# bcgsc/abyss

Measured on AMD Instinct MI355X. Metric: Mk-mers/s inserted+extended (abyss-bloom-dbg, k=64); unitig bit-exact, higher is better.
Workload: dtype u64

## Files before the change

abyss_amd/csrc/abg_engine.h:

```cpp
#pragma once
#include "abg_walk.h"

#include <algorithm>
#include <chrono>
#include <cstdio>
#include <cstdlib>
#include <cstring>
#include <functional>
#include <future>
#include <string>
#include <type_traits>
#include <vector>

namespace abg {

struct Failure { int code; std::string msg; };
constexpr int FAIL_INVAL = -1, FAIL_NOMEM = -3, FAIL_INTERNAL = -4;
[[noreturn]] inline void fail_now(int code, const std::string& msg) { throw Failure{ code, msg }; }
inline std::string strf(const char* fmt, unsigned long long a = 0, unsigned long long b = 0)
{
	char buf[256];
	snprintf(buf, sizeof buf, fmt, a, b);
	return buf;
}

struct Config {
	uint32_t k = 0, nh = 4, kc = 2, trim = 0;
	uint64_t counters = 0;
	uint32_t cascade_levels = 0;
	std::string spaced_seed;
	uint64_t insert_batch_kmers = 1ull << 24;
	uint32_t claim_log2 = 30;
	uint32_t drain_threshold = 1u << 12;
	uint64_t compact_threshold = 1u << 20;
	bool async_load = true;
	bool tiled_insert = true;
	bool benign_sharers = true;
	uint32_t cls_debug_skip = 0;
	bool cls_archive = true;
	uint32_t cls_archive_max_mb = 16384;
	bool sorted_overflow = true;
	bool cosettle = true;
	uint32_t cosettle_passes = 6;
	uint32_t cosettle_log2 = 24;
	uint32_t walk_slots = 4096;
	uint32_t tb_cap = 512;
	uint32_t buf_cap = 1u << 16;
	uint64_t pool_cap = 1ull << 28;
	uint32_t rec_cap = 1u << 22;
	uint32_t wtab_log2 = 26;
	uint32_t wtab_log2_max = 31;
	uint32_t cend_log2 = 20;
	uint64_t p2_first_batch = 65536;
	uint64_t p2_max_batch = 1ull << 22;
	uint32_t p2_growth = 2;
	uint32_t p2_crowded = 1u << 18;
	uint32_t p2_starved_growth = 2;
	uint32_t p2_starved = 6144;
	uint32_t slice_filter = 0;
	bool solid_plane = true;
	uint32_t classify_slots = 0;
	uint32_t cls_both_max_mb = 1024;
	bool cls_both = true;
	bool prefetch_classify = true;
	uint32_t memo_log2 = 0;
	bool memo = true;
	uint32_t p2_max_candidates = 1u << 18;
	uint32_t t_tags = 1024;
	uint32_t commit_incremental = 1;
	uint32_t commit_dirty_max = 4096;
	uint32_t commit_dirty_log2 = 26;
	uint32_t guide_stride = 4;
	uint32_t guide_log2_max = 31;
	bool guide_seen = true;
	bool link_duplicates = true;
	bool par_commit = true;
	bool overlap_bins = true;
	bool overlap_purity = true;
	bool apply_mask = true;
	bool lead_implicit = true;
	uint32_t dist_hash_all_ranks = 2;
	uint32_t dist_route_min_ranks = 4;
	uint64_t keep_insert_scratch_bytes = 16ull << 30;
	uint64_t par_commit_max_bytes = 16ull << 30;
	int verbose = 0;
};

struct Counters {
	uint64_t solid_reads = 0, visited_reads = 0, reads_processed = 0, bases_assembled = 0,
	         contig_id = 0;
};

struct BaseCodes {
	uint8_t t[256];
	BaseCodes()
	{
		for (int i = 0; i < 256; i++) t[i] = 0xFF;
		t['A'] = t['a'] = 0; t['C'] = t['c'] = 1; t['G'] = t['g'] = 2; t['T'] = t['t'] = 3;
	}
};
template <class T>
struct NoInitAlloc : std::allocator<T> {
	template <class U> struct rebind { using other = NoInitAlloc<U>; };
	template <class U, class... A> void construct(U* p, A&&... a)
	{
		if constexpr (sizeof...(A) == 0) ::new ((void*)p) U; else ::new ((void*)p) U(std::forward<A>(a)...);
	}
};
struct HostBatch {
	std::vector<uint32_t, NoInitAlloc<uint32_t>> words;
	std::vector<uint64_t> woff{ 0 };
	std::vector<uint32_t> len;
	std::vector<uint64_t> koff{ 0 };
	void clear() { words.clear(); woff.assign(1, 0); len.clear(); koff.assign(1, 0); }
	uint64_t n() const { return len.size(); }
	void add_ascii(const char* s, uint32_t L, uint32_t k)
	{
		static const BaseCodes codes;
		uint64_t w0 = words.size();
		words.resize(w0 + (L + 15) / 16);
		uint32_t* out = words.data() + w0;
		uint32_t i = 0;
		for (; i + 16 <= L; i += 16) {
			uint32_t w = 0;
			for (uint32_t j = 0; j < 16; j++) w |= (uint32_t)(codes.t[(unsigned char)s[i + j]] & 3u) << (2 * j);
			*out++ = w;
		}
		if (i < L) {
// ... 2604 lines not shown
						both_set(e.both32, pos);
						if (e.cnt8) { const unsigned c = e.cnt8[pos]; mn = c < mn ? c : mn; }
					}
					if (e.cnt8) cov += mn;
				}
				if (cov) atomic_add_u32(&rec.coverage, cov);
			}
		}
		if (lane == 0) { e.cnt[i] = nrec; e.cnt2[i] = nins; e.cnt3[i] = bases; }
	}
};
struct FPcCover {
	ParCommit e; uint8_t* kmin; uint32_t sum;
	ABG_HDN void operator()(uint64_t i, uint32_t lane, uint32_t nlanes) const
	{
		const uint32_t c = e.c_begin + (uint32_t)i;
		if (c >= e.brk || !e.active[i]) return;
		for (uint32_t ri = e.first_rec[c]; ri != REC_END; ri = e.recs[ri].next) {
			ContigRec& rec = e.recs[ri];
			if (!rec.ins) continue;
			const uint64_t* ch = e.kh + rec.seq_off;
			const uint32_t cnk = rec.len - e.p.k + 1;
			uint32_t cov = 0;
			for (uint32_t j = lane; j < cnk; j += nlanes) {
				if (sum) { cov += kmin[rec.seq_off + j]; continue; }
				const uint64_t h = ch[j];
				unsigned mn = 255;
				for (unsigned q = 0; q < e.p.nh; q++) {
					const uint64_t pos = pos_i(e.p, h, q);
					if (pos - e.own_lo < e.own_span) { const unsigned v = e.cnt8[pos]; mn = v < mn ? v : mn; }
				}
				kmin[rec.seq_off + j] = (uint8_t)mn;
			}
			if (sum && cov) atomic_add_u32(&rec.coverage, cov);
		}
	}
};
struct FPcWrite {
	ParCommit e; uint32_t* order; uint32_t order_base; uint64_t id_base;
	ABG_HD void operator()(uint64_t i, uint32_t) const
	{
		const uint32_t c = e.c_begin + (uint32_t)i;
		if (c >= e.brk || !e.active[i]) return;
		uint32_t o = order_base + e.cnt[i];
		uint64_t id = id_base + e.cnt2[i];
		for (uint32_t ri = e.first_rec[c]; ri != REC_END; ri = e.recs[ri].next) {
			ContigRec& rec = e.recs[ri];
			order[o++] = ri;
			if (rec.ins) rec.contig_id = id++;
		}
	}
};

constexpr uint32_t CLS_SLOTS_SMALL = 65536;
template <class BE> auto classify_lanes(BE& be, int) -> decltype(be.classify_lanes()) { return be.classify_lanes(); }
template <class BE> uint32_t classify_lanes(BE&, long) { return CLS_SLOTS_SMALL; }
template <class BE> auto device_mem_free(BE& be, int) -> decltype(be.device_mem_free()) { return be.device_mem_free(); }
template <class BE> uint64_t device_mem_free(BE&, long) { return 0; }
template <class BE>
class Engine {
  public:
	Engine(BE& be, const Config& cfg) : be_(be), cfg_(cfg)
	{
		uint64_t rem = cfg_.counters % 8;
		m_ = rem ? cfg_.counters + 8 - rem : cfg_.counters;
		p_ = make_params(cfg_.k, cfg_.nh, cfg_.kc, cfg_.trim, m_);
		if (!cfg_.spaced_seed.empty()) {
			MaskTab* mt = new MaskTab;
			make_mask(cfg_.spaced_seed.c_str(), cfg_.k, *mt, p_);
			mask_d_ = (MaskTab*)be_.alloc(sizeof(MaskTab));
			be_.h2d(mask_d_, mt, sizeof(MaskTab));
			delete mt;
			p_.mask = mask_d_;
		}
		if (cfg_.cascade_levels) {
			casc_.levels = cfg_.cascade_levels;
			casc_.level_words = (m_ + 31) / 32;
			casc_.bits = (uint32_t*)be_.alloc(casc_.levels * casc_.level_words * 4);
			be_.memset(casc_.bits, 0, casc_.levels * casc_.level_words * 4);
			cnt_ = (uint8_t*)be_.alloc(8);
			vis_bytes_ = 8;
		} else {
			const uint64_t dev = be_.device_mem_bytes();
			cnt_deferred_ = cfg_.slice_filter == 1 || (cfg_.slice_filter == 0 && dev && (double)m_ * 1.3 > (double)dev * 0.9);
			if (!cnt_deferred_) {
				cnt_ = (uint8_t*)be_.alloc(m_ + 64 * (MAX_RANKS + 1));
				be_.memset(cnt_, 0, m_);
			}
			vis_bytes_ = (m_ / 8 + 4 + 3) & ~3ull;
		}
		vis_ = (uint8_t*)be_.alloc(vis_bytes_);
		be_.memset(vis_, 0, vis_bytes_);
		cstate_ = (CommitState*)be_.alloc(sizeof(CommitState));
		be_.memset(cstate_, 0, sizeof(CommitState));
		scal_ = (uint64_t*)be_.alloc(64);
	}
	~Engine()
	{
		if (BE::ITEM_GROUP_LOG2 == 0 && getenv("ABG_LEAD_COUNT"))
			fprintf(stderr, "lead_stores made=%llu skipped=%llu\n", (unsigned long long)stats_.lead_stores[0], (unsigned long long)stats_.lead_stores[1]);
		free_counters(); be_.free(vis_); if (both_) be_.free(both_); be_.free(cstate_); be_.free(scal_);
		free_archive();
		if (casc_.bits) be_.free(casc_.bits);
		if (mask_d_) be_.free(mask_d_);
		if (T_) be_.free(T_);
		if (Tk_) { be_.free(Tk_); be_.free(Tv_); }
// ... 379 lines not shown
		mark("batches");
		deliveries_wait();
		be_.sync_side();
		mark("last delivery");
		pre_n_ = 0; prefetch_ = nullptr;
		guide_.tab = nullptr;
		be_.free(result_d);
	}
	void ensure_memo()
	{
		if (!cfg_.memo) { memo_.k0 = nullptr; return; }
		if (!memo_tab_.hmin) {
			uint32_t log2 = cfg_.memo_log2;
			if (!log2) { log2 = 16; while (log2 < 26 && (1ull << log2) < m_ / 128) log2++; }
			alloc_tab(memo_tab_, log2);
			memo_valid_ = false; plane_valid_ = false;
		}
		if (!memo_valid_) {
			be_.memset(memo_tab_.hmin, 0xFF, (memo_tab_.mask + 1) * 8);
			be_.memset(memo_tab_.hmax, 0xFF, (memo_tab_.mask + 1) * 8);
			be_.memset(memo_tab_.meta, 0, (memo_tab_.mask + 1) * 8);
			memo_valid_ = true;
			memo_gen_++;
		}
		memo_ = SuccMemo{ memo_tab_.hmin, memo_tab_.hmax, memo_tab_.meta, memo_tab_.mask };
	}
	void ensure_plane()
	{
		p2_ = p_; cnt2_ = cnt_;
		if (!cfg_.solid_plane || casc_.bits || (m_ & 63)) return;
		if (!plane_) plane_ = (uint8_t*)be_.alloc((sliced_ ? (uint64_t)comm_.world * own_chunk_ : m_) / 8 + 64);
		if (!plane_valid_ && sliced_) {
			FSolidPlane f{ (const uint64_t*)(cnt_ + own_lo_), p_.kc, (uint64_t*)(plane_ + own_lo_ / 8) };
			be_.launch(own_span_ / 64, f, "solid_plane");
			std::vector<uint64_t> c(comm_.world), d(comm_.world);
			for (int q = 0; q < comm_.world; q++) { d[q] = (uint64_t)q * (own_chunk_ / 8); c[q] = own_chunk_ / 8; }
			c_all_gather_v(plane_, c.data(), d.data());
			plane_valid_ = true; cnt_partial_ = false;
		} else if (!plane_valid_) {
			FSolidPlane f{ (const uint64_t*)cnt_, p_.kc, (uint64_t*)plane_ };
			be_.launch(m_ / 64, f, "solid_plane");
			plane_valid_ = true;
		}
		p2_.solid_bits = 1; cnt2_ = plane_;
	}
	void ensure_both()
	{
		const bool want = cfg_.cls_both && p2_.solid_bits && !dist() && !sliced_ && !(m_ & 63) && m_ / 4 <= ((uint64_t)cfg_.cls_both_max_mb << 20);
		if (!want) { if (both_) { be_.free(both_); both_ = nullptr; } return; }
		if (!both_) both_ = (uint8_t*)be_.try_alloc(m_ / 4 + 64);
		if (!both_) return;
		FBothBuild f{ (const uint32_t*)plane_, (const uint32_t*)vis_, (uint64_t*)both_ };
		be_.launch(m_ / 32, f, "both_build");
	}
	uint8_t* both_ = nullptr;
	void free_archive()
	{
		if (arc_.seq) { be_.free(arc_.seq); be_.free(arc_.used); be_.free(arc_.tab); }
		arc_ = ContigArchive(); arc_valid_ = false;
	}
	void ensure_archive(const Batch& b)
	{
		const bool want = cfg_.cls_archive && !dist() && !sliced_ && !casc_.bits && b.n && use_par_commit();
		if (!want) { free_archive(); return; }
		const uint64_t nk = loaded_ops_ ? loaded_ops_ : m_ / 4;
		uint64_t cap = std::max<uint64_t>(nk / 4, 1ull << 16) + ARC_HEAD, slots = 1ull << 12;
		while (slots < cap / 2) slots <<= 1;
		const uint64_t budget = (uint64_t)cfg_.cls_archive_max_mb << 20;
		while (slots > (1ull << 12) && slots * 8 + cap > budget) { slots >>= 1; cap = std::min(cap, slots * 2); }
		if (cap >= (1ULL << ARC_POS_BITS)) cap = (1ULL << ARC_POS_BITS) - 1;
		if (arc_.seq && (arc_.cap < cap || arc_.mask + 1 < slots)) free_archive();
		if (!arc_.seq) {
			arc_.seq = (uint8_t*)be_.try_alloc(cap + ARC_PAD);
			arc_.tab = (uint64_t*)be_.try_alloc(slots * 8);
			arc_.used = (uint64_t*)be_.try_alloc(8);
			if (!arc_.seq || !arc_.tab || !arc_.used) {
				if (arc_.seq) be_.free(arc_.seq); if (arc_.tab) be_.free(arc_.tab); if (arc_.used) be_.free(arc_.used);
				arc_ = ContigArchive();
				return;
			}
			arc_.cap = cap; arc_.mask = slots - 1;
			arc_valid_ = false;
		}
		arc_.nreads = wstats_ ? wstats_ + WSTAT_CLS_COVERED : nullptr;
		if (!arc_valid_) {
			be_.memset(arc_.seq, ARC_SEP, arc_.cap + ARC_PAD);
			be_.memset(arc_.tab, 0, (arc_.mask + 1) * 8);
			const uint64_t head = ARC_HEAD;
			be_.h2d(arc_.used, &head, 8);
			arc_valid_ = true;
		}
	}
	ContigArchive arc_{}; bool arc_valid_ = false;
	uint64_t loaded_ops_ = 0;
	uint64_t ovf_seen_[2] = { 0, 0 };
	uint8_t* plane_ = nullptr; bool plane_valid_ = false;
	Params p2_; const uint8_t* cnt2_ = nullptr;

	void build_guide(const Batch& b)
	{
		guide_.tab = nullptr; guide_.seen = nullptr; guide_slots_ = 0;
		if (!cfg_.guide_stride || p_.nh > 8 || !b.n) return;
		const uint64_t sampled = (b.n + cfg_.guide_stride - 1) / cfg_.guide_stride;
		uint64_t nwords = 0;
		be_.d2h(&nwords, b.woff + b.n, 8);
		const uint64_t bases = nwords * 16, minus = b.n * (uint64_t)(p_.k - 1);
		const uint64_t kmers = (bases > minus ? bases - minus : b.n) / std::min<uint32_t>(cfg_.guide_stride, 4u);
		uint32_t log2 = 16;
// ... 851 lines not shown
		free_tab(wtab_);
		wtab_log2_++;
		alloc_tab(wtab_, wtab_log2_);
		be_.free(pool_); be_.free(kh_);
		pool_cap_ *= 2;
		pool_ = (uint8_t*)be_.alloc(pool_cap_);
		kh_ = (uint64_t*)be_.alloc(pool_cap_ * 8);
		if (cfg_.verbose)
			fprintf(stderr, "abyss_amd: walker resources grown: %u frames, %u bases, 2^%u table, %llu pool\n",
			    walk_tb_cap_, walk_buf_cap_, wtab_log2_, (unsigned long long)pool_cap_);
	}

	template <int NW>
	WalkEnv<NW> make_env(const Batch& b, uint32_t* cand_d, uint32_t* status_d, uint32_t* first_d)
	{
		WalkEnv<NW> e;
		e.p = p2_; e.cnt = cnt2_; e.batch = b; e.cand_read = cand_d; e.status = status_d; e.first_rec = first_d;
		e.tab = wtab_; e.owner_base = 0;
		e.tb_pool = (TBFrame<NW>*)tb_pool_;
		e.tbk_pool = tbk_pool_;
		e.tb_cap = walk_tb_cap_;
		e.fast = nullptr; e.fast_bytes = 0; e.dbg = dbg_; e.coop = false;
		e.la_pool = la_pool_;
		e.guide = guide_; e.bulk_pool = bulk_pool_; e.wstats = wstats_; e.memo = memo_; e.mcache = nullptr;
		e.lbuf_pool = lbuf_; e.rbuf_pool = rbuf_; e.buf_cap = walk_buf_cap_;
		e.pool = pool_; e.pool_cap = pool_cap_; e.pool_used = pool_used_;
		e.recs = recs_; e.rec_cap = rec_cap_; e.rec_used = rec_used_;
		return e;
	}

	template <int NW>
	uint32_t commit(const Batch& b, uint32_t* cand_d, uint32_t* status_d, uint32_t* first_d,
	    uint8_t* result_d, const uint64_t* rkoff_d, uint32_t c_begin, uint32_t c_end)
	{
		{
			uint32_t nrec = 0, nord = 0;
			be_.d2h(&nrec, rec_used_, 4);
			be_.d2h(&nord, order_n_, 4);
			uint64_t need = cend_count_ + 2ull * (std::min(nrec, rec_cap_) - std::min(nord, rec_cap_));
			while (need * 2 > cend_.mask + 1) grow_cend();
		}
		CommitState cs;
		cs.counters = counters_;
		cs.break_at = c_begin; cs.pad_ = 0; cs.cend_count = cend_count_;
		be_.h2d(cstate_, &cs, sizeof cs);
		{
			FPreCommit<NW> f{ p_, b, cand_d, status_d, first_d, recs_, vis_, kh_, rkh_, rkoff_d, read_flag_, c_begin, 0, ~0ULL, nullptr, nullptr, nullptr };
			be_.launch_wave(c_end - c_begin, f, "precommit");
			FPreCommitCopies fc{ status_d, first_d, recs_, read_flag_, c_begin, p_.k };
			be_.launch(c_end - c_begin, fc, "precommit");
		}
		CommitEnv<NW> e;
		e.read_flag = read_flag_;
		e.p = p_; e.b = b; e.vis32 = (uint32_t*)vis_; e.both32 = (uint32_t*)both_;
		e.cand_read = cand_d; e.status = status_d; e.first_rec = first_d;
		e.recs = recs_; e.pool = pool_; e.result = result_d;
		e.kh = kh_; e.rkh = rkh_; e.rkoff = rkoff_d;
		e.cend = cend_; e.st = cstate_;
		e.order = order_; e.order_n = order_n_;
		be_.template launch_commit<NW>(e, c_begin, c_end);
		be_.d2h(&cs, cstate_, sizeof cs);
		counters_ = cs.counters;
		cend_count_ = cs.cend_count;
		if (cs.pad_) fail_now(FAIL_INTERNAL, "contigEndKmers table overflowed");
		return cs.break_at;
	}

	template <int NW>
	uint32_t commit_par(const Batch& b, uint32_t* cand_d, uint32_t* status_d, uint32_t* first_d,
	    uint8_t* result_d, uint64_t* rkoff_d, uint32_t c_begin, uint32_t c_end)
	{
		uint32_t n = c_end - c_begin;
		const uint32_t n0 = n;
		uint32_t nrec = 0, nord = 0;
		be_.d2h(&nrec, rec_used_, 4);
		be_.d2h(&nord, order_n_, 4);
		nrec = std::min(nrec, rec_cap_);
		{
			uint64_t need = cend_count_ + 2ull * (nrec - std::min(nord, rec_cap_));
			while (need * 2 > cend_.mask + 1) grow_cend();
		}
		const bool part = dist();
		uint8_t* part_buf = part ? (uint8_t*)be_.alloc((uint64_t)n + nrec + 64) : nullptr;
		uint8_t* part_c = part_buf; uint8_t* part_r = part ? part_buf + n : nullptr;
		uint32_t* nfirst = part ? nullptr : (uint32_t*)be_.alloc(n * 4ull + 4);
		if (nfirst) be_.memset(nfirst, 0, n * 4ull);
		{
			if (part) be_.memset(part_buf, 1, (uint64_t)n + nrec);
			FPreCommit<NW> f{ p_, b, cand_d, status_d, first_d, recs_, vis_, kh_, rkh_, rkoff_d, read_flag_, c_begin,
				part ? own_lo_ : 0, part ? own_span_ : ~0ULL, part_c, part_r, nfirst };
			be_.launch_wave(n, f, "precommit");
			if (!part) { FPreCommitCopies fc{ status_d, first_d, recs_, read_flag_, c_begin, p_.k }; be_.launch(n, fc, "precommit"); }
			if (part) {
				c_all_reduce(part_buf, (uint64_t)n + nrec, DT_U8, OP_MIN);
				FPreCommitFin ff{ status_d, first_d, recs_, read_flag_, c_begin, p_.k, part_c, part_r };
				be_.launch(n, ff, "precommit");
			}
		}
		ParCommit e;
		e.own_lo = part ? own_lo_ : 0; e.own_span = part ? own_span_ : ~0ULL; e.part_c = part_c; e.part_r = part_r;
		e.p = p_; e.b = b; e.cand_read = cand_d; e.status = status_d; e.first_rec = first_d;
		e.recs = recs_; e.pool = pool_; e.result = result_d; e.kh = kh_; e.rkh = rkh_; e.rkoff = rkoff_d;
		e.read_flag = read_flag_; e.vis32 = (uint32_t*)vis_; e.both32 = (uint32_t*)both_; e.T = T_; e.cend = cend_; e.cnt8 = cnt_;
		if (!part) e.arc = arc_;
		e.Tk = nullptr; e.Tv = nullptr; e.Tmask = 0;
		if (t_hashed()) {
			uint64_t bases = 0;
			be_.d2h(&bases, pool_used_, 8);
			const uint64_t need = std::min<uint64_t>(bases, pool_cap_) * p_.nh + 16;
			if (!Tk_ || (T_entries_ + need) * 2 > (1ull << Tlog2_)) {
				uint32_t log2 = 20;
				while ((1ull << log2) < 2 * need) log2++;
				if (!Tk_ || log2 > Tlog2_) {
					if (Tk_) { be_.free(Tk_); be_.free(Tv_); }
					Tlog2_ = log2;
					Tk_ = (uint64_t*)be_.alloc(8ull << Tlog2_);
					Tv_ = (uint32_t*)be_.alloc(4ull << Tlog2_);
				}
				be_.memset(Tk_, 0xFF, 8ull << Tlog2_);
				be_.memset(Tv_, 0xFF, 4ull << Tlog2_);
				T_entries_ = 0;
				t_tag_ = std::min<uint32_t>(cfg_.t_tags, T_TAGS) - 1;
			}
			T_entries_ += need;
			e.T = nullptr; e.Tk = Tk_; e.Tv = Tv_; e.Tmask = (1ull << Tlog2_) - 1;
		}
		e.c_begin = c_begin; e.c_end = c_end; e.brk = c_end;
		e.off = (uint32_t*)be_.alloc((n + 1ull) * 4); e.cnt = (uint32_t*)be_.alloc(n * 4ull + 4);
		e.cnt2 = (uint32_t*)be_.alloc(n * 4ull + 4); e.cnt3 = (uint64_t*)be_.alloc(n * 8ull + 8);
		e.active = (uint8_t*)be_.alloc(n + 8ull); e.short_list = (uint32_t*)be_.alloc(nrec * 4ull + 4);
		e.scal = (uint32_t*)be_.alloc(64);
		uint32_t scal_h[8] = { 0, 0xFFFFFFFFu, 0, 0, 0, 0, 0, 0 };
		be_.h2d(e.scal, scal_h, sizeof scal_h);
		e.nfirst = nfirst;
		const bool incremental = cfg_.commit_incremental && (cfg_.commit_incremental > 1 || !t_hashed()) && !part && cfg_.commit_dirty_max > 0 && nrec > 0;
		uint32_t* dirty_buf = nullptr;
		e.dirty = nullptr; e.dirty_cap = 0; e.A = nullptr; e.A_shift = 0;
		if (incremental) {
			e.dirty_cap = (uint32_t)std::min<uint64_t>(std::min(cfg_.commit_dirty_max, 8192u), std::max(nrec, 1u));
			dirty_buf = (uint32_t*)be_.alloc(2ull * e.dirty_cap * 4 + 8);
			e.dirty = dirty_buf;
			if (!pcA_) {
				const uint32_t log2 = std::min(34u, std::max(10u, cfg_.commit_dirty_log2));
				pcA_bits_ = std::min<uint64_t>(m_, 1ull << log2);
				pcA_shift_ = pcA_bits_ < m_ ? 64 - log2 : 0;
				pcA_ = (uint32_t*)be_.alloc((pcA_bits_ + 31) / 32 * 4 + 4);
				be_.memset(pcA_, 0, (pcA_bits_ + 31) / 32 * 4 + 4);
			}
			e.A = pcA_; e.A_shift = pcA_shift_;
		}
		e.tcend = WalkTab{ nullptr, nullptr, nullptr, 0 };
		std::vector<uint32_t> c1(n), c2(n), off(n + 1ull);
		{ FPcCount f{ e }; be_.launch(n, f, "pc_count"); }
		be_.d2h(c1.data(), e.cnt, n * 4ull);
		off[0] = 0;
		for (uint32_t i = 0; i < n; i++) off[i + 1] = off[i] + c1[i];
// ... 241 lines not shown
		if (log2 == wtab_log2_) return;
		free_tab(wtab_);
		wtab_log2_ = log2;
		alloc_tab(wtab_, wtab_log2_);
		if (cfg_.verbose) fprintf(stderr, "abyss_amd: walker vertex table grown to 2^%u entries\n", wtab_log2_);
	}
	uint32_t wtab_log2_cap()
	{
		uint32_t cap = cfg_.wtab_log2_max;
		const uint64_t mem = be_.device_mem_bytes();
		while (mem && cap > cfg_.wtab_log2 && (24ull << cap) > mem / 8) cap--;
		return cap;
	}
	void clear_wtab()
	{
		be_.memset(wtab_.hmin, 0xFF, (wtab_.mask + 1) * 8);
		be_.memset(wtab_.meta, 0xFF, (wtab_.mask + 1) * 8);
	}

	struct BatchRun {
		Batch v{};
		uint64_t first = 0, n = 0;
		uint8_t* res_d = nullptr;
		std::vector<uint32_t> cand_h;
		uint32_t nc = 0;
		uint32_t* cand_d = nullptr; uint32_t* status_d = nullptr; uint32_t* first_d = nullptr;
		uint32_t* need_d = nullptr; uint32_t* need_n = nullptr; uint64_t* rkoff_d = nullptr;
		uint32_t base = 0;
		uint32_t prepped = 0, owner_next = 0, committed = 0, force = 0xFFFFFFFFu, nneed = 0, nneed_all = 0;
		bool round_started = false;
		bool predicted = false;
		bool pending = false;
		bool overflow = false, debug = false;
	};
	template <int NW>
	void assemble_nw(const Batch& b, uint8_t* result_d, uint8_t* results_host,
	    const std::function<void(const ContigOut&)>& sink)
	{
		uint64_t next = 0;
		while (next < b.n) {
			ensure_walk();
			BatchRun r;
			classify_batch<NW>(b, next, std::min<uint64_t>(p2_batch_, b.n - next), result_d, r);
			next += r.n;
			counters_.reads_processed += r.n;
			p2_batch_ = next_batch_size();
			prefetch_ = nullptr;
			if (next < b.n && !dist() && cfg_.prefetch_classify) {
				const uint64_t nf = next, nn = std::min<uint64_t>(p2_batch_, b.n - next);
				prefetch_ = [this, &b, result_d, nf, nn]() {
					if (!la_pool_c2_) la_pool_c2_ = (VKey*)be_.alloc((uint64_t)cslots_ * LA_MAX_VISITED * sizeof(VKey));
					Batch vn = b;
					vn.woff = b.woff + nf; vn.len = b.len + nf; vn.koff = b.koff + nf; vn.n = nn;
					FClassify<NW> f{ p2_, vn, 0, cnt2_, vis_, result_d + nf, la_pool_c2_, both_, arc_, cfg_.cls_debug_skip };
					be_.launch_slots_side(nn, f, cslots_, "classify");
					pre_first_ = nf; pre_n_ = nn;
				};
			}
			if (r.nc) {
				setup_batch<NW>(r);
				finish_batch<NW>(r, sink);
			}
			if (results_host) {
				be_.d2h(results_host + r.first, r.res_d, r.n);
				if (const void* left = memchr(results_host + r.first, RES_CANDIDATE, r.n)) {
					fail_now(FAIL_INTERNAL, strf("read %llu left unprocessed", (unsigned long long)((const uint8_t*)left - results_host)));
				}
			}
		}
	}

	template <int NW>
	void classify_batch(const Batch& b, uint64_t first, uint64_t n, uint8_t* result_d, BatchRun& r)
	{
		Batch v = b;
		v.woff = b.woff + first; v.len = b.len + first; v.koff = b.koff + first; v.n = n;
		uint8_t* res_d = result_d + first;
		if (!la_pool_c_) la_pool_c_ = (VKey*)be_.alloc((uint64_t)cslots_ * LA_MAX_VISITED * sizeof(VKey));
		if (pre_n_ == n && pre_first_ == first) {
			const auto t_wait = std::chrono::steady_clock::now();
			be_.sync_side();
			stats_.cls_wait_ms += std::chrono::duration<double, std::milli>(std::chrono::steady_clock::now() - t_wait).count();
			FRefilter<NW> f{ p_, v, vis_, res_d };
			be_.launch(n, f, "reclassify");
		} else if (dist()) {
			const uint64_t R = (uint64_t)comm_.world;
			std::vector<uint64_t> c(R), d(R);
			for (uint64_t q = 0; q < R; q++) { d[q] = n * q / R; c[q] = n * (q + 1) / R - d[q]; }
			FClassify<NW> f{ p2_, v, d[comm_.rank], cnt2_, vis_, res_d, la_pool_c_ };
			be_.launch_slots(c[comm_.rank], f, cslots_, "classify");
			c_all_gather_v(res_d, c.data(), d.data());
		} else {
			be_.sync_side();
			FClassify<NW> f{ p2_, v, 0, cnt2_, vis_, res_d, la_pool_c_, both_, arc_, cfg_.cls_debug_skip };
			be_.launch_slots(n, f, cslots_, "classify");
		}
		pre_n_ = 0;
		std::vector<uint8_t> res(n);
		be_.d2h(res.data(), res_d, n);
		r = BatchRun();
		uint64_t used = n;
		const uint64_t max_cand = std::min<uint64_t>(cfg_.p2_max_candidates,
		    std::max<uint64_t>(1024, (1ull << wtab_log2_cap()) / (2 * wtab_per_walker_)));
		for (const uint8_t* q = res.data(), *end = q + n; (q = (const uint8_t*)memchr(q, RES_CANDIDATE, (size_t)(end - q))) != nullptr; q++) {
			if (r.cand_h.size() >= max_cand) { used = (uint64_t)(q - res.data()); break; }
			r.cand_h.push_back((uint32_t)(q - res.data()));
		}
		uint64_t n_visited = 0;
		for (uint64_t i = 0; i < used; i++) n_visited += res[i] == RR_ALL_KMERS_VISITED;
		counters_.solid_reads += n_visited + r.cand_h.size();
		counters_.visited_reads += n_visited;
		v.n = used;
		r.v = v; r.first = first; r.n = used; r.res_d = res_d;
		r.nc = (uint32_t)r.cand_h.size();
		if (used < n) stats_.batch_cuts++;
		stats_.candidates += r.nc;
		last_candidates_ = r.nc;
	}

	template <int NW>
	void setup_batch(BatchRun& r)
	{
		const uint32_t nc = r.nc;
		const Batch& b = r.v;
		r.cand_d = (uint32_t*)be_.alloc(nc * 4ull);
		r.status_d = (uint32_t*)be_.alloc(nc * 4ull);
		r.first_d = (uint32_t*)be_.alloc(nc * 4ull);
		r.need_d = (uint32_t*)be_.alloc(nc * 4ull);
		r.need_n = (uint32_t*)be_.alloc(8);
		be_.h2d(r.cand_d, r.cand_h.data(), nc * 4ull);
		std::vector<uint32_t> len_h(nc);
		{
			uint32_t* cl = (uint32_t*)be_.alloc(nc * 4ull + 4);
			FGatherU32 f{ b.len, r.cand_d, cl };
			be_.launch(nc, f, "gather_len");
			be_.d2h(len_h.data(), cl, nc * 4ull);
			be_.free(cl);
		}
		std::vector<uint64_t> rkoff(nc + 1, 0);
		for (uint32_t i = 0; i < nc; i++) rkoff[i + 1] = rkoff[i] + (len_h[i] - p_.k + 1);
		r.rkoff_d = (uint64_t*)be_.alloc((nc + 1) * 8ull);
		be_.h2d(r.rkoff_d, rkoff.data(), (nc + 1) * 8ull);
		rkh_ = (uint64_t*)be_.alloc(std::max<uint64_t>(rkoff[nc], 1) * 8);
		read_flag_ = (uint8_t*)be_.alloc(nc);
		{
			FReadPrep<NW> f{ p_, b, r.cand_d, r.rkoff_d, rkh_, 0 };
// ... 210 lines not shown
```

abyss_amd/csrc/abg_host.h:

```cpp
#pragma once
#include "abg_engine.h"
#include "../../include/abyss_amd.h"

#include <cctype>
#include <cmath>
#include <map>
#include <string>
#include <atomic>
#include <chrono>
#include <future>
#include <memory>
#include <thread>

namespace abg {
static_assert(FAIL_NOMEM == ABG_ENOMEM && FAIL_INTERNAL == ABG_EINTERNAL, "Failure codes are the C ABI's");


struct FContainsSolid {
	Params p; const uint64_t* h0; const uint8_t* cnt; uint8_t* out;
	ABG_HD void operator()(uint64_t t, uint32_t) const { out[t] = solid_contains(p, cnt, h0[t]) ? 1 : 0; }
};
struct FExpand {
	Params p; const uint64_t* h0; uint64_t* out;
	ABG_HD void operator()(uint64_t t, uint32_t) const
// ... 23 lines not shown
	explicit Session(A&&... a) : be(std::forward<A>(a)...) {}
	~Session() { try { drain(); } catch (...) {} keep_drop(false); delete eng; }

	int create(const abg_params& p)
	{
		if (p.k < 2 || p.k > ABG_MAX_KMER) return fail(ABG_EINVAL, "k must be in 2.." + std::to_string(ABG_MAX_KMER));
		if (p.num_hashes < 1 || p.num_hashes > ABG_MAX_HASHES) return fail(ABG_EINVAL, "num_hashes must be in 1..32");
		if (p.spaced_seed && p.spaced_seed[0]) {
			std::string m(p.spaced_seed);
			if (m.size() != p.k) return fail(ABG_EINVAL, "spaced seed must be exactly k bits long");
			if (m.find_first_not_of("01") != std::string::npos) return fail(ABG_EINVAL, "spaced seed must contain only '0's or '1's");
			if (m.front() != '1' || m.back() != '1') return fail(ABG_EINVAL, "spaced seed must begin and end with '1's");
			if (!std::equal(m.begin(), m.end(), m.rbegin())) return fail(ABG_EINVAL, "spaced seed must be symmetric");
			if (m.find('0') != std::string::npos) cfg.spaced_seed = m;
		}
		cfg.k = p.k; cfg.nh = p.num_hashes; cfg.kc = p.min_cov;
		cfg.trim = (p.trim == 0xFFFFFFFFu) ? p.k : p.trim;
		cfg.counters = p.counters ? p.counters : counters_for_budget(p.bloom_bytes);
		cfg.cascade_levels = p.cascade_levels;
		cfg.slice_filter = p.slice_filter;
		if (const char* e = getenv("ABG_SLICE_FILTER")) cfg.slice_filter = (uint32_t)atoi(e);
		if (p.cascade_levels && (!p.counters || p.counters % 64)) return fail(ABG_EINVAL, "cascade mode needs `counters` = bits per level, a multiple of 64");
		if (!cfg.counters) return fail(ABG_EINVAL, "bloom_bytes / counters must be > 0");
		cfg.verbose = p.verbose;
		if (p.insert_batch_kmers) cfg.insert_batch_kmers = p.insert_batch_kmers;
		if (p.claim_log2) cfg.claim_log2 = p.claim_log2;
		if (p.walk_slots) cfg.walk_slots = p.walk_slots;
		if (p.wtab_log2) cfg.wtab_log2 = p.wtab_log2;
		if (const char* e = getenv("ABG_CLAIM_LOG2")) cfg.claim_log2 = (uint32_t)atoi(e);
		if (const char* e = getenv("ABG_INSERT_BATCH")) cfg.insert_batch_kmers = strtoull(e, 0, 10);
		if (const char* e = getenv("ABG_WALK_SLOTS")) cfg.walk_slots = (uint32_t)atoi(e);
		if (const char* e = getenv("ABG_WTAB_LOG2")) cfg.wtab_log2 = (uint32_t)atoi(e);
		if (const char* e = getenv("ABG_WTAB_LOG2_MAX")) cfg.wtab_log2_max = (uint32_t)std::max<int>(atoi(e), (int)cfg.wtab_log2);
		if (const char* e = getenv("ABG_POOL_CAP")) cfg.pool_cap = std::max<uint64_t>(1024, strtoull(e, 0, 10));
		if (const char* e = getenv("ABG_REC_CAP")) cfg.rec_cap = (uint32_t)std::max(16, atoi(e));
		if (const char* e = getenv("ABG_P2_FIRST_BATCH")) cfg.p2_first_batch = strtoull(e, 0, 10);
		if (const char* e = getenv("ABG_P2_MAX_BATCH")) cfg.p2_max_batch = strtoull(e, 0, 10);
		if (const char* e = getenv("ABG_PAR_COMMIT")) cfg.par_commit = atoi(e) != 0;
		if (const char* e = getenv("ABG_T_TAGS")) cfg.t_tags = (uint32_t)std::max(2, atoi(e));
		if (const char* e = getenv("ABG_COMMIT_INCREMENTAL")) cfg.commit_incremental = (uint32_t)std::min(2, std::max(0, atoi(e)));
		if (const char* e = getenv("ABG_COMMIT_DIRTY_MAX")) cfg.commit_dirty_max = (uint32_t)std::max(0, atoi(e));
		if (const char* e = getenv("ABG_COMMIT_DIRTY_LOG2")) cfg.commit_dirty_log2 = (uint32_t)std::min(34, std::max(10, atoi(e)));
		if (const char* e = getenv("ABG_PAR_COMMIT_MAX_GB")) cfg.par_commit_max_bytes = strtoull(e, 0, 10) << 30;
		if (const char* e = getenv("ABG_COMPACT_THRESHOLD")) cfg.compact_threshold = strtoull(e, 0, 10);
		if (const char* e = getenv("ABG_TILED")) cfg.tiled_insert = atoi(e) != 0;
		if (const char* e = getenv("ABG_DIST_ROUTE_MIN")) cfg.dist_route_min_ranks = (uint32_t)atoi(e);
		if (const char* e = getenv("ABG_BENIGN")) cfg.benign_sharers = atoi(e) != 0;
		if (const char* e = getenv("ABG_CLS_ARCHIVE")) cfg.cls_archive = atoi(e) != 0;
		if (const char* e = getenv("ABG_CLS_DEBUG_SKIP")) cfg.cls_debug_skip = (uint32_t)atoi(e);
		if (const char* e = getenv("ABG_CLS_ARCHIVE_MAX_MB")) cfg.cls_archive_max_mb = (uint32_t)std::max(0, atoi(e));
		if (const char* e = getenv("ABG_SORTED_OVERFLOW")) cfg.sorted_overflow = atoi(e) != 0;
		if (const char* e = getenv("ABG_COSETTLE")) cfg.cosettle = atoi(e) != 0;
		if (const char* e = getenv("ABG_CLS_BOTH")) cfg.cls_both = atoi(e) != 0;
		if (const char* e = getenv("ABG_CLS_BOTH_MAX_MB")) cfg.cls_both_max_mb = (uint32_t)std::max(0, atoi(e));
		if (const char* e = getenv("ABG_COSETTLE_PASSES")) cfg.cosettle_passes = (uint32_t)std::max(1, atoi(e));
		if (const char* e = getenv("ABG_COSETTLE_LOG2")) cfg.cosettle_log2 = (uint32_t)std::min(25, std::max(5, atoi(e)));
		if (const char* e = getenv("ABG_LINK_DUPS")) cfg.link_duplicates = atoi(e) != 0;
		if (const char* e = getenv("ABG_OVERLAP_PURITY")) cfg.overlap_purity = atoi(e) != 0;
		if (const char* e = getenv("ABG_LEAD_IMPLICIT")) cfg.lead_implicit = atoi(e) != 0;
		if (const char* e = getenv("ABG_APPLY_MASK")) cfg.apply_mask = atoi(e) != 0;
		if (const char* e = getenv("ABG_OVERLAP_BINS")) cfg.overlap_bins = atoi(e) != 0;
		if (const char* e = getenv("ABG_PREFETCH")) cfg.prefetch_classify = atoi(e) != 0;
		if (const char* e = getenv("ABG_ASYNC_LOAD")) cfg.async_load = atoi(e) != 0;
		if (const char* e = getenv("ABG_CLS_SLOTS")) cfg.classify_slots = (uint32_t)std::max(64, atoi(e));
		if (const char* e = getenv("ABG_SOLID_PLANE")) cfg.solid_plane = atoi(e) != 0;
		if (const char* e = getenv("ABG_MEMO")) cfg.memo = atoi(e) != 0;
		if (const char* e = getenv("ABG_P2_MAX_CANDIDATES")) cfg.p2_max_candidates = (uint32_t)std::max(1, atoi(e));
		if (const char* e = getenv("ABG_P2_STARVED_GROWTH")) cfg.p2_starved_growth = (uint32_t)std::max(2, atoi(e));
		if (const char* e = getenv("ABG_P2_STARVED")) cfg.p2_starved = (uint32_t)atoi(e);
		if (const char* e = getenv("ABG_P2_GROWTH")) cfg.p2_growth = (uint32_t)std::max(2, atoi(e));
		if (const char* e = getenv("ABG_DRAIN_THRESHOLD")) cfg.drain_threshold = (uint32_t)strtoul(e, 0, 10);
		if (const char* e = getenv("ABG_GUIDE_STRIDE")) cfg.guide_stride = (uint32_t)strtoul(e, 0, 10);
		if (const char* e = getenv("ABG_GUIDE_SEEN")) cfg.guide_seen = atoi(e) != 0;
		if (const char* e = getenv("ABG_GUIDE_LOG2_MAX")) cfg.guide_log2_max = (uint32_t)std::min(36, std::max(10, atoi(e)));
		if (!be.ok()) return fail(ABG_ENODEV, be.why());
		eng = new Engine<BE>(be, cfg);
		return ABG_OK;
	}

	int load_seqs(const char* seqs, const uint64_t* off, uint64_t n) { return load_seqs_v(1, &seqs, &off, &n); }
	int load_seqs_v(uint32_t nchunks, const char* const* seqs_v, const uint64_t* const* off_v, const uint64_t* n_v)
	{
		const uint32_t k = cfg.k;
		const double t_call = std::chrono::duration<double>(std::chrono::steady_clock::now().time_since_epoch()).count();
		const uint32_t max_piece = (uint32_t)std::min<uint64_t>(1u << 20, cfg.insert_batch_kmers + k - 1);
		struct Part { uint32_t c; uint64_t a, b; };
		std::vector<Part> plan;
		std::vector<uint64_t> base(nchunks + 1, 0);
		for (uint32_t c = 0; c < nchunks; c++) {
			base[c + 1] = base[c] + n_v[c];
			if (!n_v[c]) continue;
			const std::vector<uint64_t> cut = split_reads(off_v[c], n_v[c]);
			for (size_t t = 0; t + 1 < cut.size(); t++) plan.push_back(Part{ c, cut[t], cut[t + 1] });
		}
		const bool keeping = keep_on_ && !keep_failed_;
		std::vector<KeptPart> kparts(keeping ? plan.size() : 0);
		std::vector<uint8_t> verdict(keeping ? base[nchunks] : 0, (uint8_t)RR_UNINITIALIZED);
		std::vector<HostBatch> parts(plan.size());
		const bool timing = getenv("ABG_HOST_TIMING") != nullptr;
		const auto tnow = []() { return std::chrono::duration<double>(std::chrono::steady_clock::now().time_since_epoch()).count(); };
		const double t0 = tnow();
		run_parts(parts.size(), [&](size_t t) {
			HostBatch& hb = parts[t];
			const Part& pt = plan[t];
			const char* seqs = seqs_v[pt.c];
			const uint64_t* off = off_v[pt.c];
// ... 721 lines not shown
```

abyss_amd/csrc/abg_kernels.hip:

```cpp
#include <hip/hip_runtime.h>
#include <hip/hip_ext.h>
#include <hipcub/hipcub.hpp>
#include <rccl/rccl.h>
#include <dlfcn.h>
#include <unistd.h>

#include "abg_host.h"
#include "abg_overlap.h"

#include <chrono>
#include <map>
#include <mutex>

namespace {

template <class F>
__global__ void __launch_bounds__(256) k_foreach(F f, uint64_t n)
{
	uint64_t i = (uint64_t)blockIdx.x * blockDim.x + threadIdx.x;
	const uint64_t stride = (uint64_t)gridDim.x * blockDim.x;
	const uint32_t slot = (uint32_t)i;
	for (; i < n; i += stride) f(i, slot);
}
#ifndef ABG_CLS_WAVES
// ... 137 lines not shown
struct ProfEntry { double ms = 0; uint64_t launches = 0; };

struct HipBackend {
	static constexpr uint32_t ITEM_GROUP_LOG2 = 6;
	int device = 0;
	bool good = false;
	std::string reason;
	hipStream_t stream = nullptr;
	hipStream_t stream2 = nullptr;
	hipEvent_t ev2a = nullptr, ev2b = nullptr;
	std::string side_name;
	bool side_pending = false;
	bool profiling = false;
	std::map<std::string, ProfEntry> prof;
	uint32_t cus = 256;
	unsigned long long* ticket = nullptr;

	explicit HipBackend(int dev = 0) : device(dev)
	{
		int n = 0;
		hipError_t e = hipGetDeviceCount(&n);
		if (e != hipSuccess || n <= 0) { reason = "no HIP device available (abyss_amd has no CPU fallback)"; return; }
		if (dev < 0 || dev >= n) { reason = "HIP device ordinal out of range"; return; }
		if (hipSetDevice(dev) != hipSuccess) { reason = "hipSetDevice failed"; return; }
		hipDeviceProp_t prop;
		if (hipGetDeviceProperties(&prop, dev) == hipSuccess) cus = (uint32_t)prop.multiProcessorCount;
		if (hipStreamCreate(&stream) != hipSuccess) { reason = "hipStreamCreate failed"; return; }
		if (const char* e = getenv("ABG_MEM_LIMIT_MB")) mem_limit = (size_t)strtoull(e, 0, 10) << 20;
		if (const char* e = getenv("ABG_CLS_TICKETS")) cls_tickets = atoi(e) != 0;
		{
			int lo = 0, hi = 0;
			hipDeviceGetStreamPriorityRange(&lo, &hi);
			const char* e = getenv("ABG_SIDE_PRIORITY");
			const bool low = !e || atoi(e) != 0;
			if (hipStreamCreateWithPriority(&stream2, hipStreamNonBlocking, low ? lo : hi) != hipSuccess) { reason = "hipStreamCreate failed"; return; }
		}
		hipEventCreate(&ev2a);
		hipEventCreate(&ev2b);
		good = true;
	}
	~HipBackend()
	{
		if (ticket) free(ticket);
		if (cls_ticket_) free(cls_ticket_);
		if (pin) hipHostFree(pin);
		for (int i = 0; i < 2; i++) { if (big_pin[i]) hipHostFree(big_pin[i]); if (big_ev[i]) hipEventDestroy(big_ev[i]); }
		for (int i = 0; i < 2; i++) { if (ahead_pin[i]) hipHostFree(ahead_pin[i]); if (ahead_ev[i]) hipEventDestroy(ahead_ev[i]); if (ahead[i].dev) hipFree(ahead[i].dev); }
		for (void* q : ahead_old) hipFree(q);
		if (ahead_stream) hipStreamDestroy(ahead_stream);
		if (cub_tmp) hipFree(cub_tmp);
		drop_cache();
		prof_drain(true);
		for (auto& q : prof_free) { hipEventDestroy(q.first); hipEventDestroy(q.second); }
		if (ev2a) hipEventDestroy(ev2a);
		if (ev2b) hipEventDestroy(ev2b);
		if (stream2) hipStreamDestroy(stream2);
		if (stream) hipStreamDestroy(stream);
	}
	bool ok() const { return good; }
	std::string why() const { return reason; }
	void bind_thread() { (void)hipSetDevice(device); }
	static void check(hipError_t e, const char* what)
	{
		if (e != hipSuccess) {
			(void)hipGetLastError();
			abg::fail_now(e == hipErrorOutOfMemory ? abg::FAIL_NOMEM : abg::FAIL_INTERNAL, std::string(what) + " failed: " + hipGetErrorString(e));
		}
	}
	static constexpr size_t CACHE_MAX_BLOCK = 256ull << 20, CACHE_MAX_TOTAL = 8ull << 30;
	std::map<size_t, std::vector<void*>> cache_free;
	std::map<void*, size_t> cache_size;
	size_t cache_held = 0;
	size_t mem_limit = 0, mem_used = 0;
	std::map<void*, size_t> mem_size;
	hipError_t dev_malloc(void** p, size_t n)
	{
		if (mem_limit && mem_used + n > mem_limit) return hipErrorOutOfMemory;
		const hipError_t e = hipMalloc(p, n);
		if (e == hipSuccess && mem_limit) { mem_used += n; mem_size[*p] = n; }
		return e;
	}
	void dev_free(void* p)
	{
		if (mem_limit) { auto it = mem_size.find(p); if (it != mem_size.end()) { mem_used -= it->second; mem_size.erase(it); } }
		hipFree(p);
	}
	void* try_alloc(size_t n)
	{
		void* p = nullptr;
		hipSetDevice(device);
		if (dev_malloc(&p, n ? n : 1) != hipSuccess) { (void)hipGetLastError(); return nullptr; }
		if (getenv("ABG_MEM_DEBUG")) fprintf(stderr, "[mem] +%.2f GB (optional)\n", n / 1e9);
		return p;
	}
	void* alloc(size_t n)
	{
		void* p = nullptr;
		hipSetDevice(device);
		if (n > CACHE_MAX_BLOCK) {
			hipError_t e = dev_malloc(&p, n);
			if (e != hipSuccess) {
				(void)hipGetLastError();
				drop_cache();
				e = dev_malloc(&p, n);
			}
			if (e != hipSuccess) out_of_memory(n);
// ... 273 lines not shown
	{
		if (!n) return;
		uint64_t blocks = (n + 255) / 256;
		uint64_t cap = (uint64_t)cus * 8;
		if (blocks > cap) blocks = cap;
		launch_kernel(name, k_foreach<F>, dim3((uint32_t)blocks), dim3(256), f, n);
	}
	template <class F>
	void launch_slots(uint64_t n, F f, uint32_t slots, const char* name)
	{
		if (!n) return;
		uint64_t blocks = (n + 63) / 64;
		uint64_t cap = slots / 64 ? slots / 64 : 1;
		if (blocks > cap) blocks = cap;
		if (!cls_tickets) { launch_kernel(name, k_foreach_w<F>, dim3((uint32_t)blocks), dim3(64), f, n); return; }
		unsigned long long* t = cls_ticket(0);
		check(hipMemsetAsync(t, 0, 8, stream), "hipMemsetAsync");
		launch_kernel(name, k_foreach_wt<F>, dim3((uint32_t)blocks), dim3(64), f, n, t);
	}
	bool cls_tickets = true;
	unsigned long long* cls_ticket_ = nullptr;
	unsigned long long* cls_ticket(int side)
	{
		if (!cls_ticket_) cls_ticket_ = (unsigned long long*)alloc(256);
		return cls_ticket_ + (side ? 16 : 0);
	}
	uint32_t classify_lanes() const { return cus * 4 * ABG_CLS_WAVES * 64; }
	uint64_t device_mem_free() const
	{
		size_t fr = 0, tot = 0;
		if (hipMemGetInfo(&fr, &tot) != hipSuccess) { (void)hipGetLastError(); return 0; }
		if (mem_limit) fr = std::min(fr, mem_limit > mem_used ? mem_limit - mem_used : (size_t)0);
		return fr;
	}
	template <class F>
	void launch_slots_side(uint64_t n, F f, uint32_t slots, const char* name)
	{
		if (!n) return;
		uint64_t blocks = (n + 63) / 64;
		uint64_t cap = slots / 64 ? slots / 64 : 1;
		if (blocks > cap) blocks = cap;
		hipEventRecord(ev2a, stream);
		hipStreamWaitEvent(stream2, ev2a, 0);
		unsigned long long* t = cls_tickets ? cls_ticket(1) : nullptr;
		if (t) check(hipMemsetAsync(t, 0, 8, stream2), "hipMemsetAsync");
		hipEventRecord(ev2a, stream2);
		if (t) hipLaunchKernelGGL(k_foreach_wt<F>, dim3((uint32_t)blocks), dim3(64), 0, stream2, f, n, t);
		else hipLaunchKernelGGL(k_foreach_w<F>, dim3((uint32_t)blocks), dim3(64), 0, stream2, f, n);
		check(hipGetLastError(), name);
		hipEventRecord(ev2b, stream2);
		side_name = name;
		side_pending = true;
	}
	hipEvent_t evs0 = nullptr, evs1 = nullptr;
	bool scope_pending = false, scope_saved_prof = false;
	std::string scope_name;
	void side_scope_begin(const char* name)
	{
		if (!evs0) { hipEventCreate(&evs0); hipEventCreate(&evs1); }
		scope_name = name;
		hipEventRecord(evs0, stream);
		hipStreamWaitEvent(stream2, evs0, 0);
		std::swap(stream, stream2);
		scope_saved_prof = profiling; profiling = false;
		hipEventRecord(evs0, stream);
	}
	void side_scope_end()
	{
		hipEventRecord(evs1, stream);
		std::swap(stream, stream2);
		profiling = scope_saved_prof;
		scope_pending = true;
	}
	void wait_side_scope()
	{
		if (!scope_pending) return;
		check(hipEventSynchronize(evs1), "hipEventSynchronize");
		if (profiling) {
			float ms = 0;
			hipEventElapsedTime(&ms, evs0, evs1);
			ProfEntry& p = prof[scope_name];
			p.ms += ms;
			p.launches++;
		}
		scope_pending = false;
	}
	bool side_done() { return !side_pending || hipEventQuery(ev2b) == hipSuccess; }
	void sync_side()
	{
		if (!side_pending) return;
		check(hipEventSynchronize(ev2b), "hipEventSynchronize");
		if (profiling) {
			float ms = 0;
			hipEventElapsedTime(&ms, ev2a, ev2b);
			ProfEntry& p = prof[side_name];
			p.ms += ms;
			p.launches++;
		}
		side_pending = false;
	}
	template <class F>
	void launch_wave(uint64_t n, F f, const char* name)
	{
		if (!n) return;
		uint64_t blocks = (n + 3) / 4;
		uint64_t cap = (uint64_t)cus * 8;
// ... 614 lines not shown
```

Measured before the change: 1735.

## Skip incremental both-bitmap updates in commit; rebuild it before classify, on side stream

Commit kernels now get a null both32 pointer, so they no longer keep the packed solid/visited 'both' bitmap in sync one write at a time. The bitmap is instead marked stale and rebuilt wholesale from the plane and visited bits just before the next classify launch. For prefetched classify the rebuild runs on the side stream, ordered after the main stream. This trades scattered per-commit bitmap writes for a full m/32-element rebuild kernel per classify round, which adds bandwidth cost on large tables and depends on correct ordering against later commits.

```diff
diff --git a/abyss_amd/csrc/abg_engine.h b/abyss_amd/csrc/abg_engine.h
--- a/abyss_amd/csrc/abg_engine.h
+++ b/abyss_amd/csrc/abg_engine.h
@@ -74,6 +74,7 @@
 	uint32_t guide_log2_max = 31;
 	bool guide_seen = true;
 	bool link_duplicates = true;
+	bool both_refresh = true;
 	bool par_commit = true;
 	bool overlap_bins = true;
 	bool overlap_purity = true;
@@ -2784,6 +2785,8 @@
 	}
 };
 
+template <class BE, class F> auto be_launch_side(BE& be, uint64_t n, F f, const char* name, int) -> decltype(be.launch_side(n, f, name), void()) { be.launch_side(n, f, name); }
+template <class BE, class F> void be_launch_side(BE& be, uint64_t n, F f, const char* name, long) { be.launch(n, f, name); }
 constexpr uint32_t CLS_SLOTS_SMALL = 65536;
 template <class BE> auto classify_lanes(BE& be, int) -> decltype(be.classify_lanes()) { return be.classify_lanes(); }
 template <class BE> uint32_t classify_lanes(BE&, long) { return CLS_SLOTS_SMALL; }
@@ -3269,8 +3272,18 @@
 		if (!both_) return;
 		FBothBuild f{ (const uint32_t*)plane_, (const uint32_t*)vis_, (uint64_t*)both_ };
 		be_.launch(m_ / 32, f, "both_build");
+		both_fresh_ = true;
 	}
 	uint8_t* both_ = nullptr;
+	uint32_t* commit_both() { if (cfg_.both_refresh && both_) { both_fresh_ = false; return nullptr; } return (uint32_t*)both_; }
+	void refresh_both(bool side)
+	{
+		if (!both_ || !cfg_.both_refresh || both_fresh_) return;
+		FBothBuild f{ (const uint32_t*)plane_, (const uint32_t*)vis_, (uint64_t*)both_ };
+		if (side) be_launch_side(be_, m_ / 32, f, "both_build", 0);
+		else { be_.launch(m_ / 32, f, "both_build"); both_fresh_ = true; }
+	}
+	bool both_fresh_ = false;
 	void free_archive()
 	{
 		if (arc_.seq) { be_.free(arc_.seq); be_.free(arc_.used); be_.free(arc_.tab); }
@@ -4228,7 +4241,7 @@
 		}
 		CommitEnv<NW> e;
 		e.read_flag = read_flag_;
-		e.p = p_; e.b = b; e.vis32 = (uint32_t*)vis_; e.both32 = (uint32_t*)both_;
+		e.p = p_; e.b = b; e.vis32 = (uint32_t*)vis_; e.both32 = commit_both();
 		e.cand_read = cand_d; e.status = status_d; e.first_rec = first_d;
 		e.recs = recs_; e.pool = pool_; e.result = result_d;
 		e.kh = kh_; e.rkh = rkh_; e.rkoff = rkoff_d;
@@ -4277,7 +4290,7 @@
 		e.own_lo = part ? own_lo_ : 0; e.own_span = part ? own_span_ : ~0ULL; e.part_c = part_c; e.part_r = part_r;
 		e.p = p_; e.b = b; e.cand_read = cand_d; e.status = status_d; e.first_rec = first_d;
 		e.recs = recs_; e.pool = pool_; e.result = result_d; e.kh = kh_; e.rkh = rkh_; e.rkoff = rkoff_d;
-		e.read_flag = read_flag_; e.vis32 = (uint32_t*)vis_; e.both32 = (uint32_t*)both_; e.T = T_; e.cend = cend_; e.cnt8 = cnt_;
+		e.read_flag = read_flag_; e.vis32 = (uint32_t*)vis_; e.both32 = commit_both(); e.T = T_; e.cend = cend_; e.cnt8 = cnt_;
 		if (!part) e.arc = arc_;
 		e.Tk = nullptr; e.Tv = nullptr; e.Tmask = 0;
 		if (t_hashed()) {
@@ -4625,6 +4638,7 @@
 					if (!la_pool_c2_) la_pool_c2_ = (VKey*)be_.alloc((uint64_t)cslots_ * LA_MAX_VISITED * sizeof(VKey));
 					Batch vn = b;
 					vn.woff = b.woff + nf; vn.len = b.len + nf; vn.koff = b.koff + nf; vn.n = nn;
+					refresh_both(true);
 					FClassify<NW> f{ p2_, vn, 0, cnt2_, vis_, result_d + nf, la_pool_c2_, both_, arc_, cfg_.cls_debug_skip };
 					be_.launch_slots_side(nn, f, cslots_, "classify");
 					pre_first_ = nf; pre_n_ = nn;
@@ -4665,6 +4679,7 @@
 			c_all_gather_v(res_d, c.data(), d.data());
 		} else {
 			be_.sync_side();
+			refresh_both(false);
 			FClassify<NW> f{ p2_, v, 0, cnt2_, vis_, res_d, la_pool_c_, both_, arc_, cfg_.cls_debug_skip };
 			be_.launch_slots(n, f, cslots_, "classify");
 		}
diff --git a/abyss_amd/csrc/abg_host.h b/abyss_amd/csrc/abg_host.h
--- a/abyss_amd/csrc/abg_host.h
+++ b/abyss_amd/csrc/abg_host.h
@@ -99,6 +99,7 @@
 		if (const char* e = getenv("ABG_SORTED_OVERFLOW")) cfg.sorted_overflow = atoi(e) != 0;
 		if (const char* e = getenv("ABG_COSETTLE")) cfg.cosettle = atoi(e) != 0;
 		if (const char* e = getenv("ABG_CLS_BOTH")) cfg.cls_both = atoi(e) != 0;
+		if (const char* e = getenv("ABG_BOTH_REFRESH")) cfg.both_refresh = atoi(e) != 0;
 		if (const char* e = getenv("ABG_CLS_BOTH_MAX_MB")) cfg.cls_both_max_mb = (uint32_t)std::max(0, atoi(e));
 		if (const char* e = getenv("ABG_COSETTLE_PASSES")) cfg.cosettle_passes = (uint32_t)std::max(1, atoi(e));
 		if (const char* e = getenv("ABG_COSETTLE_LOG2")) cfg.cosettle_log2 = (uint32_t)std::min(25, std::max(5, atoi(e)));
diff --git a/abyss_amd/csrc/abg_kernels.hip b/abyss_amd/csrc/abg_kernels.hip
--- a/abyss_amd/csrc/abg_kernels.hip
+++ b/abyss_amd/csrc/abg_kernels.hip
@@ -213,6 +213,7 @@
 		drop_cache();
 		prof_drain(true);
 		for (auto& q : prof_free) { hipEventDestroy(q.first); hipEventDestroy(q.second); }
+		if (ev2c) hipEventDestroy(ev2c);
 		if (ev2a) hipEventDestroy(ev2a);
 		if (ev2b) hipEventDestroy(ev2b);
 		if (stream2) hipStreamDestroy(stream2);
@@ -592,6 +593,20 @@
 		side_name = name;
 		side_pending = true;
 	}
+	hipEvent_t ev2c = nullptr;
+	template <class F>
+	void launch_side(uint64_t n, F f, const char* name)
+	{
+		if (!n) return;
+		if (!ev2c) check(hipEventCreateWithFlags(&ev2c, hipEventDisableTiming), "hipEventCreate");
+		uint64_t blocks = (n + 255) / 256;
+		uint64_t cap = (uint64_t)cus * 8;
+		if (blocks > cap) blocks = cap;
+		check(hipEventRecord(ev2c, stream), "hipEventRecord");
+		check(hipStreamWaitEvent(stream2, ev2c, 0), "hipStreamWaitEvent");
+		hipLaunchKernelGGL(k_foreach<F>, dim3((uint32_t)blocks), dim3(256), 0, stream2, f, n);
+		check(hipGetLastError(), name);
+	}
 	hipEvent_t evs0 = nullptr, evs1 = nullptr;
 	bool scope_pending = false, scope_saved_prof = false;
 	std::string scope_name;
```

Result: no change. 1751 (median of 6 runs) (+0.9%).
